# chechaohp/gan-ode

Hardware: AMD Instinct MI355X
Metric: generated videos/sec (16-frame clips) (higher is better)
Workload: dtype f32

## Files before the change

gan-ode_amd/_lib.py:

```python
from __future__ import annotations

import ctypes as C
import os

_HERE = os.path.dirname(os.path.abspath(__file__))
LIB_PATH = os.path.join(_HERE, "lib", "libgode.so")

i32, i64, f32, ptr = C.c_int32, C.c_int64, C.c_float, C.c_void_p
cint, u32, u64 = C.c_int, C.c_uint32, C.c_uint64

ACT_NONE, ACT_RELU, ACT_LRELU, ACT_TANH_OUT = 0, 1, 2, 3
ACT_TANH, ACT_SIGMOID = 4, 5
ACT_LRELU01 = 6
EPI_RAW, EPI_TANH = 0, 1
FPROP, DGRAD = 0, 1
PACK_BORDER = 0x100
OP_IGEMM, OP_WGRAD, OP_BN_FINALIZE, OP_BN_BWD, OP_ODE_FWD, OP_ODE_BWD, OP_BCE, OP_ADAM, OP_PACK = range(1, 10)
OP_ODERNN_FWD, OP_ODERNN_BWD, OP_BN_APPLY, OP_COL2IM = 10, 11, 12, 13
OP_SDE_FWD, OP_SDE_BWD = 14, 15
OP_CDE_FWD, OP_CDE_BWD = 16, 17
OP_WGAN = 18
OP_GRU_FWD, OP_GRU_BWD = 19, 20
OP_DNOISE = 21
OP_CATEG, OP_CE = 22, 23
# ... 235 lines not shown

class SnBwdOp(_Op):
    _fields_ = [("G", ptr), ("wbar", ptr), ("u", ptr), ("v", ptr), ("sigma", ptr), ("dwbar", ptr), ("work", ptr), ("h", i32),
                ("w", i32)]
    KIND, FN = OP_SN_BWD, "gode_sn_bwd"


class FcActOp(_Op):
    _fields_ = [("y", ptr), ("b", ptr), ("out", ptr), ("M", i64), ("C", i32), ("act", i32), ("key", i64), ("layer", i32),
                ("p", f32)]
    KIND, FN = OP_FC_ACT, "gode_fc_act"


class FcActBwdOp(_Op):
    _fields_ = [("g_out", ptr), ("out", ptr), ("g_y", ptr), ("db", ptr), ("work", ptr), ("M", i64), ("C", i32), ("act", i32),
                ("key", i64), ("layer", i32), ("p", f32), ("accumulate", i32), ("pad_", i32)]
    KIND, FN = OP_FC_ACT_BWD, "gode_fc_act_bwd"


class BceProbOp(_Op):
    _fields_ = [("p", ptr), ("t", ptr), ("grad", ptr), ("loss", ptr), ("n", i64), ("gscale", f32), ("accumulate", i32)]
    KIND, FN = OP_BCE_PROB, "gode_bce_prob"


class BceTOp(_Op):
    _fields_ = [("logits", ptr), ("target", ptr), ("grad", ptr), ("loss", ptr), ("n", i64), ("gscale", f32), ("accumulate", i32)]
    KIND, FN = OP_BCE_T, "gode_bce_logits_t"


class AdamNoiseTensor(C.Structure):
    _fields_ = [("p", ptr), ("g", ptr), ("m", ptr), ("v", ptr), ("n", i64), ("noise_off", i64)]


class AdamOp(_Op):
    _fields_ = [("p", ptr), ("g", ptr), ("m", ptr), ("v", ptr), ("n", i64), ("lr", f32), ("beta1", f32),
                ("beta2", f32), ("eps", f32), ("weight_decay", f32), ("gscale", f32), ("step", i32), ("pad_", i32)]
    KIND, FN = OP_ADAM, "gode_adam_l2"


class PackOp(C.Structure):
    _fields_ = [("g", ConvGeom), ("dir", i32), ("co_canon", i32), ("w", ptr), ("wpack", ptr), ("co_perm", ptr)]
    KIND = OP_PACK


_OPS = _Op.__subclasses__()
_STRUCTS = {0: ConvGeom, REC_ADAM_NOISE: AdamNoiseTensor, OP_PACK: PackOp, **{st.KIND: st for st in _OPS}}

_PROTOS = {
    "gode_igemm_stats_rows": ([ptr], cint),
    "gode_igemm_stats_rows0": ([ptr], cint),
    "gode_igemm_stats_segments": ([ptr, i32, ptr], cint),
    "gode_igemm_model_cycles": ([ptr], C.c_double),
    "gode_igemm_family": ([ptr], cint),
    "gode_igemm_work_size": ([ptr], i64),
    "gode_pack_size": ([ptr, cint], i64),
    "gode_pack_weights": ([ptr, cint, ptr, ptr, ptr, i32, ptr], cint),
    "gode_wgrad_work_size": ([ptr], i64),
    "gode_wgrad_auto_splits": ([ptr], cint),
    "gode_bn_bwd_work_size": ([i64, i32], i64),
    "gode_ode_bwd_work_size": ([i32], i64),
    "gode_odernn_bwd_work_size": ([i32], i64),
    "gode_odernn_sync_size": ([i32], i64),
    "gode_sde_bwd_work_size": ([i32], i64),
    "gode_cde_sync_size": ([i32], i64),
    "gode_cde_state_size": ([i32, i32], i64),
    "gode_cde_bwd_work_size": ([i32], i64),
    "gode_gru_bwd_work_size": ([i32], i64),
    "gode_ode_fwd_multi": ([ptr, i32, ptr], cint),
    "gode_ode_bwd_multi": ([ptr, i32, ptr], cint),
    "gode_odernn_fwd_multi": ([ptr, i32, ptr], cint),
    "gode_odernn_bwd_multi": ([ptr, i32, ptr], cint),
    "gode_gru_fwd_multi": ([ptr, i32, ptr], cint),
    "gode_gru_bwd_multi": ([ptr, i32, ptr], cint),
    "gode_chstats_rows": ([i64], cint),
    "gode_cbn_bwd_work_size": ([i32, i32, i32, i32], i64),
    "gode_gres_out_bwd_work_size": ([i32, i32, i32, i32, i32, i32], i64),
    "gode_fc_act_bwd_work_size": ([i64, i32], i64),
    "gode_dropout_mask": ([ptr, i64, u64, u32, f32, ptr], cint),
    "gode_scale": ([ptr, ptr, i64, f32, cint, ptr], cint),
    "gode_adam_multi": ([ptr, i32, i64, f32, f32, f32, f32, f32, f32, i32, ptr], cint),
    "gode_adam_multi_dev": ([ptr, i32, i64, f32, f32, f32, f32, f32, ptr, ptr], cint),
    "gode_adam_noise_multi": ([ptr, i32, i64, f32, f32, f32, f32, f32, f32, i32, u64, u32, u32, f32, ptr], cint),
    "gode_adam_noise_multi_dev": ([ptr, i32, i64, f32, f32, f32, f32, f32, ptr, u64, u32, f32, ptr], cint),
    "gode_param_noise": ([ptr, i64, u64, u32, u32, i64, f32, i32, ptr], cint),
    "gode_dnoise_normals": ([ptr, i64, u64, u32, u32, u32, i64, i32, ptr], cint),
    "gode_ode_step_chunks": ([ptr, i64], i64),
    "gode_ode_step": ([ptr, i32, i64, i32, f32, f32, f32, f32, f32, ptr, ptr], cint),
    "gode_axpy_multi": ([ptr, i32, i64, f32, ptr, ptr, f32, ptr, ptr, ptr], cint),
    "gode_run": ([ptr, ptr, i32, ptr], cint),
    "gode_version": (None, cint),
    "gode_sizeof": ([cint], cint),
}

EXPORTS = [st.FN for st in _OPS] + list(_PROTOS)

_lib = None


def lib():
    global _lib
    if _lib is not None:
        return _lib
    if not os.path.exists(LIB_PATH):
        raise RuntimeError(f"{LIB_PATH} is missing: build it with `python __graft_entry__.py` "
                           "(hipcc --offload-arch=gfx950); there is no CPU or PyTorch fallback")
    L = C.CDLL(LIB_PATH)
# ... 65 lines not shown
```

gan-ode_amd/csrc/igemm.hip:

```cpp
#include <stdlib.h>
#include "common.h"
#include "conv_geom.h"
#include "igemm_plan.h"

int gode_launch_conv_patch_fprop(const gode_igemm_op* op, const int64_t* gs, hipStream_t st);

struct IgemmArgs {
  IgemmGeom G;
  const float* src;
  const float* w;
  float* out;
  const float* scale;
  const float* shift;
  float* stats;
  int32_t gsN, gsD, gsH, gsW, gsC;
  int32_t act, epilogue;
  int32_t MB, NB, xcd_mode;
  int32_t tapskip, dmajor;
  int32_t stagger;
  int32_t ksplit, slabs_per_split;
  float* work;
  int32_t out_numel;
  int32_t stats_rows;
  uint32_t src_bytes, w_bytes;
  int32_t ntab;
  int32_t tile0[GODE_MAX_PHASES + 1];
};

__device__ __forceinline__ void igemm_block_id(const IgemmArgs& a, int& mblk, int& nblk, int& phase, int& split) {
  if (a.ntab > 0) {
    const int id = blockIdx.x;
    int p = 0;
    while (p + 1 < a.ntab && id >= a.tile0[p + 1]) ++p;
    const int t = id - a.tile0[p], NB = a.NB, mb = (a.tile0[p + 1] - a.tile0[p]) / NB;
    const int grp = t / (8 * NB), r = t - grp * 8 * NB, rest = mb - grp * 8;
    if (rest >= 8) { mblk = grp * 8 + (r & 7); nblk = r >> 3; }
    else { mblk = grp * 8 + r % rest; nblk = r / rest; }
    phase = p; split = 0;
    return;
  }
  const int MB = a.MB, NC = a.NB * a.G.nphase;
  split = blockIdx.x / (MB * NC);
  const int id = blockIdx.x - split * (MB * NC);
  int combo;
  if (a.xcd_mode == 1) {
    const int x = id & 7, j = id >> 3;
    if ((NC & 7) == 0) { combo = x + 8 * (j / MB); mblk = j % MB; }
    else { const int parts = 8 / NC; combo = x % NC; mblk = j * parts + x / NC; }
  } else if (a.xcd_mode == 2) {
    const int x = id & 7, j = id >> 3;
    combo = j % NC; mblk = (j / NC) * 8 + x;
  } else if (a.xcd_mode == 3) {
    const int x = id & 7, j = id >> 3;
    combo = j % NC; mblk = x * (MB >> 3) + j / NC;
  } else {
    mblk = id % MB; combo = id / MB;
  }
  nblk = combo % a.NB; phase = combo / a.NB;
}

template <int WM, int WN, int TM, int TN, bool VEC>
__global__ void __launch_bounds__(WM* WN * 64) igemm_kernel(const IgemmArgs a) {
  constexpr int NT = WM * WN * 64, BM = WM * TM * 32, BN = WN * TN * 32, LDK = 36;
  constexpr int RPP = NT / 8;
  constexpr int AP = BM / RPP, BP = BN / RPP;
  static_assert(BM % RPP == 0 && BN % RPP == 0, "tile/loader mismatch");
  constexpr int BUF = (BM + BN) * LDK;
  __shared__ __attribute__((aligned(16))) float smem[2 * BUF + BM * 5];
  int* rowinfo = reinterpret_cast<int*>(smem + 2 * BUF);
  int* outoff = rowinfo + BM * 4;

  const PhaseGeom& P = a.G.ph[blockIdx.z];
  const int mblk = blockIdx.x, nblk = blockIdx.y;
  if (mblk * BM >= P.M) return;
  const int tid = threadIdx.x, lane = tid & 63, wave = tid >> 6;
  const int wm = wave / WN, wn = wave % WN;
  const int Cg = a.G.Cg, Ncols = a.G.Ncols;

  for (int r = tid; r < BM; r += NT) {
    const int m = mblk * BM + r;
    int base = -1, bd = 0, bh = 0, bw = 0, oo = -1;
    if (m < P.M) {
      const int qw = m % P.Mw; int t = m / P.Mw;
      const int qh = t % P.Mh; t /= P.Mh;
      const int qd = t % P.Md; const int img = t / P.Md + P.img0;
      base = img * a.gsN;
      bd = qd * a.G.Sd + P.Od; bh = qh * a.G.Sh + P.Oh; bw = qw * a.G.Sw + P.Ow;
      oo = (((img * a.G.Xd + qd * a.G.OSd + P.Pd) * a.G.Xh + qh * a.G.OSh + P.Ph) * a.G.Xw + qw * a.G.OSw + P.Pw) *
           Ncols;
    }
    rowinfo[r * 4 + 0] = base; rowinfo[r * 4 + 1] = bd; rowinfo[r * 4 + 2] = bh; rowinfo[r * 4 + 3] = bw;
// ... 809 lines not shown
  const float neg = gode_act_neg_slope(a.act);
  const bool xf = a.scale != nullptr;
  const int64_t wave_id = (int64_t)blockIdx.x * 4 + (threadIdx.x >> 6), nwaves = (int64_t)gridDim.x * 4;
  for (int64_t m0 = wave_id * ppw; m0 < P.M; m0 += nwaves * ppw) {
    const int m = (int)m0 + sub;
    if (m >= P.M) continue;
    const uint32_t t1 = fdiv((uint32_t)m, d.dMw[0]), qw = m - t1 * P.Mw;
    const uint32_t t2 = fdiv(t1, d.dMh[0]), qh = t1 - t2 * P.Mh;
    const uint32_t img = fdiv(t2, d.dMd[0]), qd = t2 - img * P.Md;
    const int bd = (int)qd * a.G.Sd + P.Od, bh = (int)qh * a.G.Sh + P.Oh, bw = (int)qw * a.G.Sw + P.Ow;
    f32x4 acc = {0.f, 0.f, 0.f, 0.f};
    int k = 0;
    for (int jd = 0; jd < P.Td; ++jd)
      for (int jh = 0; jh < P.Th; ++jh)
        for (int jw = 0; jw < P.Tw; ++jw) {
          const int id = bd + a.G.J * jd, ih = bh + a.G.J * jh, iw = bw + a.G.J * jw;
          const bool ok = (unsigned)id < (unsigned)a.G.Gd && (unsigned)ih < (unsigned)a.G.Gh && (unsigned)iw < (unsigned)a.G.Gw;
          const int off = (int)img * a.gsN + id * a.gsD + ih * a.gsH + iw * a.gsW;
          for (int c = 0; c < Cg; ++c, ++k) {
            float v = 0.f;
            if (ok) {
              v = a.src[off + c * a.gsC];
              if (xf) v = v * a.scale[c] + a.shift[c];
              v = fmaxf(v, v * neg);
            }
            const f32x4 w = *reinterpret_cast<const f32x4*>(wl + k * Ncols + c4);
            acc[0] += v * w[0]; acc[1] += v * w[1]; acc[2] += v * w[2]; acc[3] += v * w[3];
          }
        }
    const int oo = ((((int)img * a.G.Xd + (int)qd * a.G.OSd + P.Pd) * a.G.Xh + (int)qh * a.G.OSh + P.Ph) * a.G.Xw +
                    (int)qw * a.G.OSw + P.Pw) * Ncols;
    if (a.epilogue == GODE_EPI_TANH) { acc[0] = tanhf(acc[0]); acc[1] = tanhf(acc[1]); acc[2] = tanhf(acc[2]); acc[3] = tanhf(acc[3]); }
    *reinterpret_cast<f32x4*>(a.out + oo + c4) = acc;
  }
}

extern "C" int gode_igemm_stats_rows0(const gode_igemm_op* op) {
  IgemmPlan P;
  const int rc = igemm_make_plan(op, &P);
  return rc ? rc : P.rows0;
}

extern "C" double gode_igemm_model_cycles(const gode_igemm_op* op) {
  IgemmPlan P;
  return igemm_make_plan(op, &P) ? -1.0 : P.cycles;
}

extern "C" int gode_igemm_family(const gode_igemm_op* op) {
  IgemmPlan P;
  const int rc = igemm_make_plan(op, &P);
  return rc ? rc : P.family;
}

extern "C" int gode_igemm_stats_segments(const gode_igemm_op* op, int32_t split_images, int32_t* seg) {
  if (!op || !seg || op->groups == 2 || op->border || split_images <= 0 || split_images >= op->g.N) return GODE_E_ARG;
  IgemmPlan P;
  const int rc = igemm_make_plan(op, &P);
  if (rc) return rc;
  if (P.ksplit > 1) {
    const int64_t per_img = (int64_t)P.G.Xd * P.G.Xh * P.G.Xw;
    const int64_t b = (int64_t)split_images * per_img;
    if (b % SPLITK_ROWS != 0) return GODE_E_SHAPE;
    seg[0] = 0; seg[1] = (int32_t)(b / SPLITK_ROWS); seg[2] = P.stats_rows;
    return 1;
  }
  const int bm = tile_bm(P.tile);
  for (int i = 0; i < P.G.nphase; ++i) {
    const PhaseGeom& Ph = P.G.ph[i];
    const int64_t per_img = (int64_t)Ph.Md * Ph.Mh * Ph.Mw;
    const int64_t b = (int64_t)split_images * per_img;
    if (Ph.M != (int64_t)op->g.N * per_img) return GODE_E_SHAPE;
    if (b % bm != 0) return GODE_E_SHAPE;
    seg[3 * i] = Ph.row0; seg[3 * i + 1] = Ph.row0 + (int32_t)(b / bm); seg[3 * i + 2] = Ph.row0 + gode_ceil_div(Ph.M, bm);
  }
  return P.G.nphase;
}

extern "C" int gode_igemm_stats_rows(const gode_igemm_op* op) {
  IgemmPlan P;
  const int rc = igemm_make_plan(op, &P);
  return rc ? rc : P.stats_rows;
}

extern "C" int64_t gode_igemm_work_size(const gode_igemm_op* op) {
  IgemmPlan P;
  const int rc = igemm_make_plan(op, &P);
  if (rc) return rc;
  return P.ksplit > 1 ? (int64_t)P.ksplit * P.positions * P.G.Ncols : 0;
}

template <int TILE>
static int launch(IgemmArgs& A, const IgemmPlan& P, bool vec, hipStream_t st) {
  constexpr IgemmTile T = IGEMM_TILES[TILE];
  constexpr int WM = T.WM, WN = T.WN, TM = T.TM, TN = T.TN;
  dim3 grid(P.max_mblk, gode_ceil_div(A.G.Ncols, T.bn), A.G.nphase), block(WM * WN * 64);
  const bool fast = vec && P.fast;
  if (P.ksplit > 1 && (!fast || A.work == nullptr)) return GODE_E_ARG;
  if (fast) {
    static const char* senv = getenv("GODE_IGEMM_STAGGER");
    A.stagger = senv ? atoi(senv) : 0;
#ifndef GODE_ABLATION_BUILD
    if (A.stagger < 0) A.stagger = 0;
#endif
    const dim3 g1(P.ntab > 0 ? P.tile0[P.ntab] : P.MB * P.NB * A.G.nphase * P.ksplit);
    const bool has_xf = A.scale != nullptr || A.act != GODE_ACT_NONE;
    const bool glds = !has_xf && A.src_bytes != 0 && A.w_bytes != 0;
// ... 8 lines not shown
                           dim3(256), 0, st, A.work, A.out, A.stats, P.positions, A.G.Ncols, P.ksplit, A.epilogue);
      else
        hipLaunchKernelGGL(igemm_splitk_reduce_kernel, dim3(gode_ceil_div(P.positions, SPLITK_ROWS)), dim3(256), 0, st, A.work, A.out,
                           A.stats, P.positions, A.G.Ncols, P.ksplit, A.epilogue);
    }
  }
  else if (vec) hipLaunchKernelGGL((igemm_kernel<WM, WN, TM, TN, true>), grid, block, 0, st, A);
  else hipLaunchKernelGGL((igemm_kernel<WM, WN, TM, TN, false>), grid, block, 0, st, A);
  GODE_LAUNCH_CHECK();
  return 0;
}

static PwArgs pw_args(const IgemmArgs& A, int lanes_per_position) {
  PwArgs D; D.a = A; D.lpp = lanes_per_position;
  for (int i = 0; i < A.G.nphase; ++i) {
    D.dMw[i] = make_fastdiv((uint32_t)A.G.ph[i].Mw); D.dMh[i] = make_fastdiv((uint32_t)A.G.ph[i].Mh);
    D.dMd[i] = make_fastdiv((uint32_t)A.G.ph[i].Md);
  }
  return D;
}

extern "C" int gode_igemm(const gode_igemm_op* op, void* stream) {
  if (!op || !op->src || !op->wpack || !op->out) return GODE_E_ARG;
  IgemmPlan P;
  int rc = igemm_make_plan(op, &P);
  if (rc) return rc;
  if (P.max_mblk == 0) return 0;
  const IgemmGeom& G = P.G;
  int64_t gs[5];
  if (gode_strides_are_channels_last(op->gs)) {
    gs[4] = 1; gs[3] = G.Cg; gs[2] = (int64_t)G.Gw * gs[3]; gs[1] = (int64_t)G.Gh * gs[2]; gs[0] = (int64_t)G.Gd * gs[1];
  } else {
    for (int i = 0; i < 5; ++i) gs[i] = op->gs[i];
  }
  int64_t span = 1 + (int64_t)(op->g.N - 1) * gs[0] + (int64_t)(G.Gd - 1) * gs[1] + (int64_t)(G.Gh - 1) * gs[2] +
                 (int64_t)(G.Gw - 1) * gs[3] + (int64_t)(G.Cg - 1) * gs[4];
  int64_t outn = (int64_t)op->g.N * G.Xd * G.Xh * G.Xw * G.Ncols;
  for (int i = 0; i < 5; ++i) if (gs[i] < 0) return GODE_E_ARG;
  if (span >= (1ll << 31) || outn >= (1ll << 31)) return GODE_E_SHAPE;
  if (((uintptr_t)op->wpack % 16) != 0 || (op->scale == nullptr) != (op->shift == nullptr)) return GODE_E_ARG;
  hipStream_t st = (hipStream_t)stream;
  if (P.family == IGEMM_PATCH_FPROP) {
    const int pr = gode_launch_conv_patch_fprop(op, gs, st);
    if (pr != 0) return pr < 0 ? pr : 0;
  }
  IgemmArgs A;
  A.G = G;
  A.src = op->src; A.w = op->wpack; A.out = op->out; A.scale = op->scale; A.shift = op->shift; A.stats = op->stats;
  A.gsN = (int)gs[0]; A.gsD = (int)gs[1]; A.gsH = (int)gs[2]; A.gsW = (int)gs[3]; A.gsC = (int)gs[4];
  A.act = op->act; A.epilogue = op->epilogue;
  A.stagger = 0;
  A.tapskip = P.tapskip; A.dmajor = P.dmajor; A.stats_rows = P.stats_rows;
  A.ksplit = P.ksplit; A.slabs_per_split = P.slabs_per_split;
  A.MB = P.MB; A.NB = P.NB; A.xcd_mode = P.xcd_mode; A.ntab = P.ntab;
  for (int i = 0; i <= GODE_MAX_PHASES; ++i) A.tile0[i] = P.tile0[i];
  A.src_bytes = span * 4 < (1ll << 31) ? (uint32_t)(span * 4) : 0u;
  A.w_bytes = gode_pack_floats(G) * 4 < (1ll << 31) ? (uint32_t)(gode_pack_floats(G) * 4) : 0u;
  A.work = op->work; A.out_numel = (int32_t)outn;
  const bool vec = P.vec && ((uintptr_t)op->src % 16) == 0 &&
                   (op->scale == nullptr || ((uintptr_t)op->scale % 16 == 0 && (uintptr_t)op->shift % 16 == 0));
  int maxM = 0, minK = 1 << 30;
  for (int i = 0; i < G.nphase; ++i) {
    if (G.ph[i].M > maxM) maxM = G.ph[i].M;
    if (G.ph[i].K < minK) minK = G.ph[i].K;
  }
  if (P.family == IGEMM_POINTWISE && vec) {
    const int lpp = G.Cg / 4;
    const bool one_tap = G.nphase == 1 && G.ph[0].K == G.Cg;
    const PwArgs D = pw_args(A, lpp);
    int64_t blocks = ((int64_t)maxM + (64 / lpp) * 4 * 8 - 1) / ((64 / lpp) * 4 * 8);
    if (blocks > (one_tap ? 4096 : 2048)) blocks = one_tap ? 4096 : 2048;
    if (one_tap && G.Ncols == 1 && lpp <= 16) {
      const int64_t its = ((int64_t)maxM + (64 / lpp) * PW1_U - 1) / ((64 / lpp) * PW1_U), per_wave = (its + 8191) / 8192;
      const dim3 g1((unsigned)((its + 4 * per_wave - 1) / (4 * per_wave)));
      if (lpp == 16) hipLaunchKernelGGL(conv_pointwise1_kernel<16>, g1, dim3(256), 0, st, D);
      else if (lpp == 8) hipLaunchKernelGGL(conv_pointwise1_kernel<8>, g1, dim3(256), 0, st, D);
      else hipLaunchKernelGGL(conv_pointwise1_kernel<4>, g1, dim3(256), 0, st, D);
    }
    else if (one_tap) hipLaunchKernelGGL(conv_pointwise_kernel<true>, dim3((int)blocks, 1), dim3(256), 0, st, D);
    else hipLaunchKernelGGL(conv_pointwise_kernel<false>, dim3((int)blocks, G.nphase), dim3(256), 0, st, D);
  } else if (P.family == IGEMM_SMALLK && ((uintptr_t)op->out % 16) == 0) {
    const int nl = G.Ncols / 4;
    const PwArgs D = pw_args(A, nl);
    int64_t blocks = ((int64_t)maxM + (64 / nl) * 4 * 4 - 1) / ((64 / nl) * 4 * 4);
    if (blocks > 4096) blocks = 4096;
    hipLaunchKernelGGL(conv_smallk_kernel, dim3((int)blocks), dim3(256), 0, st, D);
  } else if (P.family == IGEMM_DOT && vec) {
    DotArgs D; D.a = A; D.dCg = make_fastdiv((uint32_t)G.Cg);
    D.per_block = (maxM <= 256 && minK >= 4096) ? 1 : 4;
    hipLaunchKernelGGL(conv_dot_kernel, dim3(D.per_block == 1 ? maxM : gode_ceil_div(maxM, 4), G.nphase), dim3(256), 0, st, D);
  } else {
    static int (*const launchers[IGEMM_TILE_IDS])(IgemmArgs&, const IgemmPlan&, bool, hipStream_t) = {
        nullptr, launch<TILE_128x128>, launch<TILE_128x64>, launch<TILE_128x32>, launch<TILE_64x64>, nullptr, launch<TILE_256x128>};
    return launchers[P.tile](A, P, vec, st);
  }
  GODE_LAUNCH_CHECK();
  return 0;
}

struct PackArgs {
  IgemmGeom G;
  gode_conv_geom g;
  int dir;
  const float* w;
  float* wp;
  const int32_t* co_perm;
};
// ... 213 lines not shown
```

gan-ode_amd/csrc/igemm_plan.h:

```cpp
#pragma once
#include <stdio.h>
#include <stdlib.h>
#include "conv_geom.h"

#define IGEMM_MAX_LIVE_TAPS 64
#define SPLITK_ROWS 16
#define PW_MAXW 4096

enum { TILE_128x128 = 1, TILE_128x64 = 2, TILE_128x32 = 3, TILE_64x64 = 4, TILE_256x128 = 6, IGEMM_TILE_IDS = 7 };
struct IgemmTile { int bm, bn, WM, WN, TM, TN; double cps; int resident; double eff2; };
constexpr IgemmTile igemm_tile(int WM, int WN, int TM, int TN, double cps, int resident, double eff2) {
  return IgemmTile{WM * TM * 32, WN * TN * 32, WM, WN, TM, TN, cps, resident, eff2};
}
static constexpr IgemmTile IGEMM_TILES[IGEMM_TILE_IDS] = {
    igemm_tile(0, 0, 0, 0, 0.0, 0, 0.0),
    igemm_tile(2, 2, 2, 2, 4096.0, 2, 0.76),
    igemm_tile(2, 2, 2, 1, 2048.0, 3, 0.76),
    igemm_tile(4, 1, 1, 1, 1024.0, 4, 0.62),
    igemm_tile(2, 2, 1, 1, 1024.0, 4, 0.70),
    igemm_tile(0, 0, 0, 0, 0.0, 0, 0.0),
    igemm_tile(4, 2, 2, 2, 8192.0, 1, 0.785)};

static bool tile_exists(int tile) { return tile > 0 && tile < IGEMM_TILE_IDS && IGEMM_TILES[tile].bm != 0; }
static int tile_bm(int tile) { return IGEMM_TILES[tile].bm; }
// ... 98 lines not shown
      if (cyc < best * 0.97) { best = cyc; best_tile = t; best_k = k; }
    }
  }
  *cycles_out = best;
  if (live_taps) {
    const int64_t t128 = count_tiles(G, TILE_128x128), t64 = count_tiles(G, TILE_64x64);
    if (t128 < 256 && G.Ncols >= 64 && min_slabs == max_slabs) {
      int k = (int)((1152 + t64 / 2) / t64);
      if (k < 1) k = 1;
      while (k > 1 && (min_slabs / k < 8 || out_bytes * k > 192e6)) --k;
      best_tile = TILE_64x64; best_k = k;
    }
  }
  *tile_out = best_tile;
  *sp_out = split_k(op, G, max_slabs, best_k);
}

static bool border_table(const gode_igemm_op* op, const IgemmGeom& G, IgemmGeom* B) {
  if (!op->border || op->dir != GODE_DGRAD || op->groups == 2 || G.fullk || igemm_wants_tapskip(op, G)) return false;
  return gode_build_igemm_geom_border(op->g, op->dir, B) == 0 && B->border != 0;
}

#define BORDER_LOSS 1.06
static void choose_border(const IgemmGeom& B, int* tile_out, double* cycles_out) {
  static const int tiles[2] = {TILE_128x64, TILE_64x64};
  double best = 1e300; int best_tile = TILE_128x64;
  for (int ti = 0; ti < 2; ++ti) {
    const int t = tiles[ti], bm = tile_bm(t), bn = tile_bn(t);
    if (bn >= 2 * B.Ncols && bn > 32) continue;
    const double cps = IGEMM_TILES[t].cps, eff = IGEMM_TILES[t].eff2;
    const int resident = IGEMM_TILES[t].resident;
    if (3 * count_tiles(B, t) < 4 * 256 * (int64_t)resident) continue;
    double work = 0;
    for (int i = 0; i < B.nphase; ++i)
      work += (double)gode_ceil_div(B.ph[i].M, bm) * gode_ceil_div(B.Ncols, bn) * (4000.0 + (B.ph[i].K >> 5) * cps / eff);
    const double cyc = BORDER_LOSS * work / 256.0;
    if (cyc < best) { best = cyc; best_tile = t; }
  }
  *tile_out = best_tile; *cycles_out = best;
}

enum { IGEMM_GEMM = 0, IGEMM_PATCH_FPROP = 1, IGEMM_POINTWISE = 2, IGEMM_SMALLK = 3, IGEMM_DOT = 4 };

struct IgemmPlan {
  IgemmGeom G;
  int32_t family;
  int32_t tile;
  int32_t vec, fast;
  int32_t ksplit, slabs_per_split, positions;
  int32_t max_mblk, stats_rows, rows0;
  int32_t tapskip, dmajor;
  int32_t xcd_mode, MB, NB;
  int32_t ntab, tile0[GODE_MAX_PHASES + 1];
  double cycles;
};

static int thin_family(const gode_igemm_op* op, const IgemmGeom& G, bool vec) {
  if (op->tile != 0 || op->stats != nullptr || op->groups == 2) return IGEMM_GEMM;
  if (op->dir == GODE_FPROP && !op->scale && !op->shift && op->act == GODE_ACT_NONE && op->epilogue == GODE_EPI_RAW && op->g.Ci <= 4 &&
      op->g.Co >= 32 && G.ph[0].K >= 8)
    return IGEMM_PATCH_FPROP;
  int maxM = 0, minK = 1 << 30, maxK = 0; bool kp_ok = true;
  for (int i = 0; i < G.nphase; ++i) {
    if (G.ph[i].M > maxM) maxM = G.ph[i].M;
    if (G.ph[i].K < minK) minK = G.ph[i].K;
    if (G.ph[i].Kp > maxK) maxK = G.ph[i].Kp;
    kp_ok = kp_ok && G.ph[i].Kp == G.ph[i].K;
  }
  const int lpp = G.Cg / 4, nl = G.Ncols / 4;
  const bool one_tap = G.nphase == 1 && G.ph[0].K == G.Cg;
  if (vec && kp_ok && G.Ncols <= 4 && G.Ncols * maxK <= PW_MAXW && maxM >= (one_tap ? 4096 : 65536) &&
      (lpp == 4 || lpp == 8 || lpp == 16 || lpp == 32 || lpp == 64))
    return IGEMM_POINTWISE;
  if (G.nphase == 1 && G.ph[0].K <= 4 && G.Ncols % 4 == 0 && G.Ncols <= 128 && maxM >= 2048 && (nl == 4 || nl == 8 || nl == 16 || nl == 32))
    return IGEMM_SMALLK;
  if (vec && kp_ok && G.Ncols <= 4 && maxM <= 16384 && minK >= 512) return IGEMM_DOT;
  return IGEMM_GEMM;
}

static void plan_grid_order(const gode_igemm_op* op, IgemmPlan* P) {
  const IgemmGeom& G = P->G;
  P->MB = 0; P->NB = 0; P->xcd_mode = 0; P->ntab = 0;
  for (int i = 0; i <= GODE_MAX_PHASES; ++i) P->tile0[i] = 0;
  if (!P->fast) return;
  const int MB = P->max_mblk, NB = gode_ceil_div(G.Ncols, tile_bn(P->tile)), NC = NB * G.nphase;
  P->MB = MB; P->NB = NB;
  static const char* xenv = getenv("GODE_IGEMM_XCD");
  const int force = xenv ? atoi(xenv) : -1;
  const int64_t wbytes = gode_pack_floats(G) * 4;
  const bool ok1 = (NC % 8 == 0) || (NC < 8 && 8 % NC == 0 && MB % (8 / NC) == 0);
  const bool ok2 = MB % 8 == 0;
  const int64_t in_bytes = (int64_t)op->g.N * G.Gd * G.Gh * G.Gw * G.Cg * 4;
  int mode = ok2 ? (wbytes * 8 < 3 * in_bytes ? 3 : 0) : 0;
  if (P->dmajor > 0) mode = ok2 ? 2 : (ok1 ? 1 : 0);
  if (force == 0) mode = 0;
  if (force == 1 && ok1) mode = 1;
  if (force == 2 && ok2) mode = 2;
  if (force == 3 && ok2) mode = 3;
  P->xcd_mode = mode;
  if (G.border) {
    P->ntab = G.nphase;
    for (int i = 0; i < G.nphase; ++i) P->tile0[i + 1] = P->tile0[i] + gode_ceil_div(G.ph[i].M, tile_bm(P->tile)) * NB;
    for (int i = G.nphase + 1; i <= GODE_MAX_PHASES; ++i) P->tile0[i] = P->tile0[G.nphase];
  }
}

static int igemm_make_plan(const gode_igemm_op* op, IgemmPlan* P) {
  if (!op || (op->tile != 0 && !tile_exists(op->tile))) return GODE_E_ARG;
  IgemmGeom& G = P->G;
  int rc = gode_build_igemm_geom(op->g, op->dir, &G);
  if (rc) return rc;
  P->tapskip = igemm_wants_tapskip(op, G);
  P->dmajor = P->tapskip ? op->g.N : 0;
  IgemmGeom B;
  const bool can_border = border_table(op, G, &B);
  const bool grouped = op->groups == 2;
  if (grouped) {
    if (op->dir != GODE_FPROP || op->g.N % 2 != 0 || G.nphase != 1) return GODE_E_ARG;
    G.ph[1] = G.ph[0];
    G.ph[0].M /= 2; G.ph[1].M = G.ph[0].M; G.ph[1].img0 = op->g.N / 2;
    G.nphase = 2;
  } else if (op->groups != 0 && op->groups != 1) return GODE_E_ARG;
  P->vec = strides_allow_vec(op, G);
  int tile; SplitPlan sp; double cyc = -1.0;
  bool take_border = false;
  if (op->tile == 0 && fast_geometry(G) && G.Ncols > 4 && P->vec) {
    choose_fast(op, G, &tile, &sp, &cyc);
    if (can_border && fast_geometry(B) && sp.ksplit == 1) {
      int tb; double cb;
      choose_border(B, &tb, &cb);
      if (cb < 0.97 * cyc) { take_border = true; tile = tb; cyc = cb; }
    }
    static const bool sweeping = getenv("GODE_IGEMM_SWEEP") != nullptr;
    const char* fenv = sweeping ? getenv("GODE_IGEMM_FORCE") : nullptr;
    int fk = 0, min_slabs, max_slabs;
    if (fenv && sscanf(fenv, "%d,%d", &tile, &fk) == 2) {
      if (!tile_exists(tile)) return GODE_E_ARG;
      slab_range(G, &min_slabs, &max_slabs);
      sp = split_k(op, G, max_slabs, fk);
      take_border = can_border && fk <= 1;
    }
  } else {
    tile = pick_tile(G, op->tile);
    sp = plan_split(op, G, tile);
    if (can_border && sp.ksplit == 1 && op->tile != 0) {
      const int tb = pick_tile(B, op->tile);
      const SplitPlan sb = plan_split(op, B, tb);
      if (sb.ksplit == 1) { take_border = true; tile = tb; sp = sb; }
    }
  }
  if (take_border) G = B;
  if (grouped && sp.ksplit > 1 && (sp.positions / 2) % SPLITK_ROWS != 0) {
    sp.ksplit = 1; sp.slabs_per_split = 0;
  }
  const int bm = tile_bm(tile);
  int r0 = 0, mx = 0;
  for (int i = 0; i < G.nphase; ++i) {
    G.ph[i].row0 = r0;
    const int mb = gode_ceil_div(G.ph[i].M, bm);
    r0 += mb;
    if (mb > mx) mx = mb;
  }
  P->tile = tile; P->ksplit = sp.ksplit; P->slabs_per_split = sp.slabs_per_split; P->positions = sp.positions;
  P->max_mblk = mx;
  P->stats_rows = sp.ksplit > 1 ? gode_ceil_div(sp.positions, SPLITK_ROWS) : r0;
  P->rows0 = !grouped ? P->stats_rows : (sp.ksplit > 1 ? P->stats_rows / 2 : G.ph[1].row0);
  P->cycles = grouped ? -1.0 : cyc;
  P->fast = P->vec && fast_geometry(G);
  P->family = thin_family(op, G, P->vec);
  plan_grid_order(op, P);
  return 0;
}
```

gan-ode_amd/engine.py:

```python
from __future__ import annotations

import ctypes as C
import os
from dataclasses import dataclass
from typing import List, Optional, Sequence

import numpy as np
import torch

from . import _lib as L


def make_geom(N, Ci, Co, xi, yo, k, s, p) -> L.ConvGeom:
    return L.ConvGeom(N, Ci, Co, xi[0], xi[1], xi[2], yo[0], yo[1], yo[2], k[0], k[1], k[2], s[0], s[1], s[2],
                      p[0], p[1], p[2])


def conv_out(i, k, s, p):
    return (i + 2 * p - k) // s + 1


def dptr(t: Optional[torch.Tensor]):
    return None if t is None else t.data_ptr()


def stream_ptr():
    return torch.cuda.current_stream().cuda_stream


@dataclass
class LayerSpec:
    geom: L.ConvGeom
    fwd_dir: int
    act: int
    has_bn: bool
    epilogue: int = L.EPI_RAW
    co_perm: Optional[torch.Tensor] = None
    noise: bool = False

    def out_dims(self):
        g = self.geom
        if self.fwd_dir == L.FPROP:
            return (g.N, g.Do, g.Ho, g.Wo, g.Co)
        return (g.N, g.Di, g.Hi, g.Wi, g.Ci)

    def in_dims(self):
        g = self.geom
        if self.fwd_dir == L.FPROP:
            return (g.N, g.Di, g.Hi, g.Wi, g.Ci)
        return (g.N, g.Do, g.Ho, g.Wo, g.Co)


@dataclass
class LayerParams:
    weight: torch.Tensor
    gamma: Optional[torch.Tensor] = None
    beta: Optional[torch.Tensor] = None
    running_mean: Optional[torch.Tensor] = None
    running_var: Optional[torch.Tensor] = None
    num_batches_tracked: Optional[torch.Tensor] = None


def _contig_strides(dims):
    n, d, h, w, c = dims
    return (d * h * w * c, h * w * c, w * c, c, 1)


class ConvStack:

    def __init__(self, specs: Sequence[LayerSpec], params: Sequence[LayerParams], device, owns_input: bool,
                 momentum=0.1, eps=1e-5, pack_cache: Optional[dict] = None, groups: int = 1, split_images: int = 0,
                 split_order: int = 0, two_lane_backward: bool = False):
        self.specs, self.params, self.device = list(specs), list(params), device
        self.groups = groups
        self.two_lane = bool(two_lane_backward)
        self._lane_stream = None
        self.split, self.split_order = int(split_images), int(split_order)
        if self.split and (groups != 1 or not owns_input or not (0 < self.split < specs[0].geom.N)):
            raise ValueError("split ConvStack: plan-owned input, one launch group, 0 < split_images < N")
        self._G2 = groups == 2 or self.split > 0
        self._last_parts = False
        if groups not in (1, 2) or (groups == 2 and (owns_input or specs[0].fwd_dir != L.FPROP or specs[0].has_bn
                                                     or specs[0].geom.N % 2)):
            raise ValueError("grouped ConvStack: two groups, Conv stack, caller-owned input, no BatchNorm on layer 0")
        self.nl = len(specs)
        self.noisy = any(s.noise for s in specs)
        if self.noisy and (owns_input or self.split):
            raise ValueError("instance noise: caller-owned input, no split stack")
        self.momentum, self.eps = momentum, eps
        self.busy = False
        self.generation = 0
        self._fwd_training = True
        self.pack_cache = pack_cache if pack_cache is not None else {}
        lib = L.lib()
        f32 = dict(dtype=torch.float32, device=device)
        self.x_in = torch.zeros(specs[0].in_dims(), **f32) if owns_input else None
        self.x0n = torch.empty(specs[0].in_dims(), **f32) if specs[0].noise else None
        self.y = [torch.empty(s.out_dims(), **f32) for s in specs[:-1]]
        self.a = [torch.empty(s.out_dims(), **f32) if self._materialize(l) else None for l, s in enumerate(specs[:-1])]
        self.out_dims = specs[-1].out_dims()
        self.wpack_f, self.wpack_b = [], [None] * self.nl
        self.stats, self.stat_rows = [], []
        self.mean, self.invstd, self.scale, self.shift = [], [], [], []
        self._two_f, self._two_b, self._rows_ab = {}, {}, {}
        self._border = self._border_layers() if os.environ.get("GODE_BORDER_SPLIT", "1") != "0" else {}
        for l, s in enumerate(specs):
            bord = l in self._border
            n = lib.gode_pack_size(C.byref(s.geom), s.fwd_dir | (L.PACK_BORDER if bord else 0))
            if n <= 0:
                raise RuntimeError(f"bad geometry for pack ({n})")
            self.wpack_f.append(self._shared_pack(l, "border" if bord else s.fwd_dir, n))
            C_out = s.out_dims()[4]
            two = self._two_f[l] = bool(self.split) and 0 < l < self.nl - 1 and self._two_launches(s.geom, s.fwd_dir)
            if s.has_bn:
                probe = L.IgemmOp(g=s.geom, dir=s.fwd_dir, tile=0, groups=groups, border=1 if bord else 0)
                if two:
                    ra, rb = (lib.gode_igemm_stats_rows(C.byref(L.IgemmOp(g=self._part_geom(s.geom, n), dir=s.fwd_dir, tile=0)))
                              for n in (self.split, s.geom.N - self.split))
                    rows = ra + rb if ra > 0 and rb > 0 else -1
                    self._rows_ab[l] = (ra, rb)
                else:
                    rows = lib.gode_igemm_stats_rows(C.byref(probe))
                if rows <= 0:
                    raise RuntimeError(f"layer {l}: no partial-statistics layout for this geometry ({rows})")
                ncols = self._ncols(s)
                self.stat_rows.append(rows)
                self.stats.append(torch.empty(rows * 2 * ncols, **f32))
                ng = 2 if self._G2 else 1
                self.mean.append(torch.empty(ng * C_out, **f32)); self.invstd.append(torch.empty(ng * C_out, **f32))
                self.scale.append(torch.empty(ng * C_out, **f32)); self.shift.append(torch.empty(ng * C_out, **f32))
                if self.split and not two:
                    seg = (C.c_int32 * 24)()
                    nseg = lib.gode_igemm_stats_segments(C.byref(probe), self.split, seg)
                    if nseg <= 0:
                        raise ValueError(f"layer {l}: the statistics rows do not split at image {self.split} ({nseg})")
                    self.__dict__.setdefault("_segs", {})[l] = (nseg, list(seg))
            else:
                self.stat_rows.append(0); self.stats.append(None)
                self.mean.append(None); self.invstd.append(None); self.scale.append(None); self.shift.append(None)
        self._ig_work = None
        self._fwd = {}
        self._bwd = {}
        self.g = None
        self._param_ptrs = None

    def _shared_pack(self, l, direction, n):
        key = ("buf", l, direction)
        buf = self.pack_cache.get(key)
        if buf is None or buf.numel() != n or buf.device != torch.device(self.device):
            buf = self.pack_cache[key] = torch.empty(n, dtype=torch.float32, device=self.device)
            self.pack_cache.pop(("ver", l, direction), None)
        return buf

    def _attach_work(self, igemm_ops):
        lib = L.lib()
        need = max([lib.gode_igemm_work_size(C.byref(op)) for op in igemm_ops] + [0])
        if need > 0:
            if self._ig_work is None or self._ig_work.numel() < need:
                self._ig_work = torch.empty(need, dtype=torch.float32, device=self.device)
                for prog_ops in getattr(self, "_all_igemm", []):
                    for op in prog_ops:
                        op.work = self._ig_work.data_ptr()
            for op in igemm_ops:
                op.work = self._ig_work.data_ptr()
        self.__dict__.setdefault("_all_igemm", []).append(list(igemm_ops))

    def _run_stale_packs(self, packs, st):
        stale = []
# ... 175 lines not shown
                wp = self._shared_pack(l, "head_gemm", n)
                packs.append((l, "head_gemm", L.PackOp(g=hg, dir=L.DGRAD, co_canon=0, w=dptr(p.weight), wpack=dptr(wp),
                                                       co_perm=dptr(s.co_perm))))
                g = s.geom
                if getattr(self, "_head_cols", None) is None:
                    self._head_cols = torch.empty(hg.N * g.kh * g.kw * g.Ci, dtype=torch.float32, device=self.device)
                if self._last_parts:
                    pix, Cs = g.Ho * g.Wo, sc.numel() // 2
                    for n, img0, k in ((self.split, 0, 0), (g.N - self.split, self.split, 1)):
                        pg = self._part_geom(hg, n * pix)
                        ops.append(L.IgemmOp(g=pg, dir=L.DGRAD, act=act, epilogue=L.EPI_RAW, tile=0,
                                             src=src.data_ptr() + 4 * img0 * pix * g.Co, wpack=dptr(wp),
                                             out=self._head_cols.data_ptr() + 4 * img0 * pix * g.kh * g.kw * g.Ci,
                                             scale=sc.data_ptr() + 4 * Cs * k, shift=sh.data_ptr() + 4 * Cs * k))
                else:
                    ops.append(L.IgemmOp(g=hg, dir=L.DGRAD, act=act, epilogue=L.EPI_RAW, tile=0, src=dptr(src), wpack=dptr(wp),
                                         out=dptr(self._head_cols), scale=dptr(sc), shift=dptr(sh)))
                c2i = L.Col2imOp(cols=dptr(self._head_cols), out=None, N=g.N, Hi=g.Ho, Wi=g.Wo, Ho=g.Hi, Wo=g.Wi, C=g.Ci,
                                 kh=g.kh, kw=g.kw, sh=g.sh, sw=g.sw, ph=g.ph, pw=g.pw, epilogue=s.epilogue)
                ops.append(c2i)
                patch["last"] = c2i
                if l == 0:
                    raise RuntimeError("a one-layer stack cannot use the GEMM + col2im head")
                continue
            want_stats = s.has_bn and training
            if self._last_parts and l == self.nl - 1:
                per_in, per_out, Cs = int(np.prod(s.in_dims()[1:])), int(np.prod(s.out_dims()[1:])), sc.numel() // 2
                pair = []
                for n, img0, k in ((self.split, 0, 0), (s.geom.N - self.split, self.split, 1)):
                    pair.append(L.IgemmOp(g=self._part_geom(s.geom, n), dir=s.fwd_dir, act=act, epilogue=s.epilogue, tile=0,
                                          src=src.data_ptr() + 4 * img0 * per_in, wpack=dptr(self.wpack_f[l]), out=None,
                                          scale=sc.data_ptr() + 4 * Cs * k, shift=sh.data_ptr() + 4 * Cs * k))
                ops += pair
                patch["last"], patch["last2"] = pair[0], (pair[1], 4 * self.split * per_out)
                continue
            if self._two_f.get(l):
                ra = self._rows_ab[l][0] if s.has_bn else 0
                per_in, per_out = int(np.prod(s.in_dims()[1:])), int(np.prod(s.out_dims()[1:]))
                for n, img0, st_off in ((self.split, 0, 0), (s.geom.N - self.split, self.split, ra * 2 * self._ncols(s))):
                    ops.append(L.IgemmOp(g=self._part_geom(s.geom, n), dir=s.fwd_dir, act=act, epilogue=s.epilogue, tile=0,
                                         src=src.data_ptr() + 4 * img0 * per_in, wpack=dptr(self.wpack_f[l]),
                                         out=self.y[l].data_ptr() + 4 * img0 * per_out, scale=dptr(sc), shift=dptr(sh),
                                         stats=self.stats[l].data_ptr() + 4 * st_off if want_stats else None, groups=0))
                op = None
            else:
                op = L.IgemmOp(g=s.geom, dir=s.fwd_dir, act=act, epilogue=s.epilogue, tile=0, src=dptr(src),
                               wpack=dptr(self.wpack_f[l]), out=dptr(self.y[l]) if l < self.nl - 1 else None,
                               scale=dptr(sc), shift=dptr(sh),
                               stats=dptr(self.stats[l]) if want_stats else None,
                               groups=2 if (G2 and s.has_bn) else 0)
                if l in self._border:
                    packs[-1] = (l, "border", L.PackOp(g=s.geom, dir=L.DGRAD | L.PACK_BORDER, co_canon=0, w=dptr(p.weight),
                                                       wpack=dptr(self.wpack_f[l]), co_perm=dptr(s.co_perm)))
                    op.border = 1
                ops.append(op)
            if l == 0:
                patch["first"] = op
            if l == self.nl - 1:
                patch["last"] = op
            if s.has_bn:
                rows0 = lib.gode_igemm_stats_rows0(C.byref(op)) if G2 else 0
                fin = L.BnFinalizeOp(stats=dptr(self.stats[l]), rows=self.stat_rows[l], ncols=self._ncols(s),
                                     C=s.out_dims()[4], count=self._count(l) // self.groups, gamma=dptr(p.gamma),
                                     beta=dptr(p.beta), running_mean=dptr(p.running_mean),
                                     running_var=dptr(p.running_var),
                                     num_batches_tracked=dptr(p.num_batches_tracked), mean=dptr(self.mean[l]),
                                     invstd=dptr(self.invstd[l]), scale=dptr(self.scale[l]),
                                     shift=dptr(self.shift[l]), momentum=self.momentum, eps=self.eps,
                                     training=1 if training else 0, groups=self.groups if G2 else 0, rows0=rows0)
                if self.split:
                    per_img = self._count(l) // s.geom.N
                    fin.groups, fin.order = 2, self.split_order
                    fin.count, fin.count1 = per_img * self.split, per_img * (s.geom.N - self.split)
                    if self._two_f.get(l):
                        ra, rb = self._rows_ab[l]
                        fin.rows, fin.rows1 = ra, rb
                        fin.stats1 = self.stats[l].data_ptr() + 4 * ra * 2 * self._ncols(s)
                    else:
                        nseg, seg = self._segs[l]
                        fin.nseg = nseg
                        for k in range(3 * nseg):
                            fin.seg[k] = seg[k]
                ops.append(fin)
            if l < self.nl - 1 and self.a[l] is not None:
                d = s.out_dims()
                M = d[0] * d[1] * d[2] * d[3]
                M0 = M // 2 if (G2 and s.has_bn) else ((M // d[0]) * self.split if (self.split and s.has_bn) else 0)
                if self.specs[l + 1].noise:
                    ops.append(self._noise_op(noise, l, dptr(self.scale[l]), dptr(self.shift[l]), M // 2 if G2 else 0))
                    continue
                ops.append(L.BnApplyOp(y=dptr(self.y[l]), out=dptr(self.a[l]), scale=dptr(self.scale[l]),
                                       shift=dptr(self.shift[l]), M=M, C=d[4], act=s.act, M0=M0))
        patch["packs"] = packs
        self._attach_work([op for op in ops if isinstance(op, L.IgemmOp)])
        return L.Program(ops), patch

    def _noise_op(self, noise, l, scale, shift, M0):
        d = self.specs[l].out_dims()
        op = L.DnoiseOp(x=dptr(self.y[l]), out=dptr(self.a[l]), scale=scale, shift=shift, M=d[0] * d[1] * d[2] * d[3],
                        C=d[4], act=self.specs[l].act, M0=M0, layer=l + 1)
        noise.append((op, d[1] * d[2] * d[3] * d[4], 0, None))
        return op

    @staticmethod
    def _patch_noise(patch, noise, inputs):
        seed = int(noise["seed"]) & 0xFFFFFFFFFFFFFFFF
        seed = seed - (1 << 64) if seed >= 1 << 63 else seed
# ... 308 lines not shown
```

include/gode.h:

```cpp
#ifndef GODE_H
#define GODE_H
#include <stdint.h>
#ifdef __cplusplus
extern "C" {
#endif

#define GODE_VERSION 105

enum { GODE_OK = 0, GODE_E_ARG = -1, GODE_E_SHAPE = -2, GODE_E_KIND = -3 };
enum { GODE_ACT_NONE = 0, GODE_ACT_RELU = 1, GODE_ACT_LRELU = 2,
       GODE_ACT_TANH_OUT = 3 ,
       GODE_ACT_TANH = 4, GODE_ACT_SIGMOID = 5 ,
       GODE_ACT_LRELU01 = 6  };
enum { GODE_EPI_RAW = 0, GODE_EPI_TANH = 1 };
enum { GODE_FPROP = 0, GODE_DGRAD = 1 };
enum { GODE_PACK_BORDER = 0x100 };

typedef struct gode_conv_geom {
  int32_t N, Ci, Co;
  int32_t Di, Hi, Wi;
  int32_t Do, Ho, Wo;
  int32_t kd, kh, kw;
  int32_t sd, sh, sw;
  int32_t pd, ph, pw;
} gode_conv_geom;

typedef struct gode_igemm_op {
  gode_conv_geom g;
  int32_t dir, act, epilogue, tile;
  const float* src;
  const float* wpack;
  float* out;
  const float* scale;
  const float* shift;
  float* stats;
  int64_t gs[5];
  float* work;
  int32_t groups;
  int32_t border;
} gode_igemm_op;
int gode_igemm(const gode_igemm_op* op, void* stream);
int64_t gode_igemm_work_size(const gode_igemm_op* op);
int gode_igemm_stats_rows(const gode_igemm_op* op);
int gode_igemm_stats_rows0(const gode_igemm_op* op);
int gode_igemm_stats_segments(const gode_igemm_op* op, int32_t split_images, int32_t* seg);
double gode_igemm_model_cycles(const gode_igemm_op* op);
int gode_igemm_family(const gode_igemm_op* op);
int64_t gode_pack_size(const gode_conv_geom* g, int dir);
int gode_pack_weights(const gode_conv_geom* g, int dir, const float* w, float* wpack, const int32_t* co_perm,
                      int32_t co_canon, void* stream);

typedef struct gode_wgrad_op {
  gode_conv_geom g;
  int32_t act, xform_on_y, splits, accumulate;
  const float* x;
  const float* y;
  const float* scale;
  const float* shift;
  float* work;
  float* dw;
  const int32_t* co_perm; int64_t co_canon;
  int64_t xs[5];
} gode_wgrad_op;
int gode_wgrad(const gode_wgrad_op* op, void* stream);
int64_t gode_wgrad_work_size(const gode_wgrad_op* op);
int gode_wgrad_auto_splits(const gode_conv_geom* g);

typedef struct gode_bn_finalize_op {
  const float* stats; int32_t rows, ncols, C; int64_t count;
  const float* gamma; const float* beta;
  float* running_mean; float* running_var; int64_t* num_batches_tracked;
  float* mean; float* invstd; float* scale; float* shift;
  float momentum, eps; int32_t training, pad_;
  int32_t groups, rows0;
  int32_t nseg, order; int64_t count1; int32_t seg[24];
  const float* stats1; int32_t rows1, pad3_;
} gode_bn_finalize_op;
int gode_bn_finalize(const gode_bn_finalize_op* op, void* stream);

typedef struct gode_bn_apply_op {
  const float* y; float* out; const float* scale; const float* shift; int64_t M; int32_t C, act;
  int64_t M0;
} gode_bn_apply_op;
int gode_bn_apply(const gode_bn_apply_op* op, void* stream);

typedef struct gode_col2im_op {
  const float* cols; float* out;
  int32_t N, Hi, Wi, Ho, Wo, C, kh, kw, sh, sw, ph, pw;
  int32_t epilogue, pad_;
  int32_t Di, Do, kd, sd, pd, pad2_;
} gode_col2im_op;
int gode_col2im(const gode_col2im_op* op, void* stream);

typedef struct gode_bn_bwd_op {
  float* g; const float* y; int64_t M; int32_t C, act;
  const float* gamma; const float* mean; const float* invstd; const float* scale; const float* shift;
  float* dgamma; float* dbeta; float* work; int32_t accumulate, eval_mode;
  const float* gin;
  int32_t groups, pad2_;
  int64_t M0;
// ... 328 lines not shown
```

Baseline: 37580.

## Force border-split igemm when dead taps are significant and interleave phase classes

Adds a border=2 mode that is chosen per layer from the fraction of dead taps and the tile count relative to resident slots. In that mode the planner takes the border (tap-skipping) decomposition unconditionally instead of only when the cycle model predicts a gain. It also reorders the phases into classes with matching shapes and interleaves the spatial residues inside each grid segment. The intent is to skip the zero-tap work in transposed convolutions and keep the grid balanced. The risk is overriding the cost model where the border split is slower, and it adds more indexing arithmetic to the block-id mapping.

```diff
diff --git a/gan-ode_amd/_lib.py b/gan-ode_amd/_lib.py
--- a/gan-ode_amd/_lib.py
+++ b/gan-ode_amd/_lib.py
@@ -311,6 +311,8 @@
     "gode_igemm_stats_segments": ([ptr, i32, ptr], cint),
     "gode_igemm_model_cycles": ([ptr], C.c_double),
     "gode_igemm_family": ([ptr], cint),
+    "gode_igemm_dead_taps": ([ptr], C.c_double),
+    "gode_igemm_launch_info": ([ptr, ptr], cint),
     "gode_igemm_work_size": ([ptr], i64),
     "gode_pack_size": ([ptr, cint], i64),
     "gode_pack_weights": ([ptr, cint, ptr, ptr, ptr, i32, ptr], cint),
diff --git a/gan-ode_amd/csrc/igemm.hip b/gan-ode_amd/csrc/igemm.hip
--- a/gan-ode_amd/csrc/igemm.hip
+++ b/gan-ode_amd/csrc/igemm.hip
@@ -23,20 +23,14 @@
   int32_t out_numel;
   int32_t stats_rows;
   uint32_t src_bytes, w_bytes;
-  int32_t ntab;
+  int32_t ntab, interleave;
   int32_t tile0[GODE_MAX_PHASES + 1];
 };
 
 __device__ __forceinline__ void igemm_block_id(const IgemmArgs& a, int& mblk, int& nblk, int& phase, int& split) {
   if (a.ntab > 0) {
-    const int id = blockIdx.x;
-    int p = 0;
-    while (p + 1 < a.ntab && id >= a.tile0[p + 1]) ++p;
-    const int t = id - a.tile0[p], NB = a.NB, mb = (a.tile0[p + 1] - a.tile0[p]) / NB;
-    const int grp = t / (8 * NB), r = t - grp * 8 * NB, rest = mb - grp * 8;
-    if (rest >= 8) { mblk = grp * 8 + (r & 7); nblk = r >> 3; }
-    else { mblk = grp * 8 + r % rest; nblk = r / rest; }
-    phase = p; split = 0;
+    igemm_border_block(blockIdx.x, a.ntab, a.tile0, a.NB, a.interleave, mblk, nblk, phase);
+    split = 0;
     return;
   }
   const int MB = a.MB, NC = a.NB * a.G.nphase;
@@ -952,6 +946,29 @@
   return rc ? rc : P.family;
 }
 
+extern "C" double gode_igemm_dead_taps(const gode_igemm_op* op) {
+  if (!op) return 0.0;
+  gode_igemm_op flagged = *op;
+  flagged.border = 1;
+  IgemmGeom G, B;
+  if (gode_build_igemm_geom(op->g, op->dir, &G) || !border_table(&flagged, G, &B)) return 0.0;
+  double plain = 0, live = 0;
+  for (int i = 0; i < G.nphase; ++i) plain += (double)G.ph[i].M * G.ph[i].K;
+  for (int i = 0; i < B.nphase; ++i) live += (double)B.ph[i].M * B.ph[i].K;
+  return plain > 0 ? 1.0 - live / plain : 0.0;
+}
+
+extern "C" int gode_igemm_launch_info(const gode_igemm_op* op, int32_t* info) {
+  if (!info) return GODE_E_ARG;
+  IgemmPlan P;
+  const int rc = igemm_make_plan(op, &P);
+  if (rc) return rc;
+  info[0] = P.G.border != 0; info[1] = P.tile;
+  info[2] = P.ntab > 0 ? P.tile0[P.ntab] : (int32_t)count_tiles(P.G, P.tile) * P.ksplit;
+  info[3] = 256 * IGEMM_TILES[P.tile].resident;
+  return 0;
+}
+
 extern "C" int gode_igemm_stats_segments(const gode_igemm_op* op, int32_t split_images, int32_t* seg) {
   if (!op || !seg || op->groups == 2 || op->border || split_images <= 0 || split_images >= op->g.N) return GODE_E_ARG;
   IgemmPlan P;
@@ -1066,7 +1083,7 @@
   A.stagger = 0;
   A.tapskip = P.tapskip; A.dmajor = P.dmajor; A.stats_rows = P.stats_rows;
   A.ksplit = P.ksplit; A.slabs_per_split = P.slabs_per_split;
-  A.MB = P.MB; A.NB = P.NB; A.xcd_mode = P.xcd_mode; A.ntab = P.ntab;
+  A.MB = P.MB; A.NB = P.NB; A.xcd_mode = P.xcd_mode; A.ntab = P.ntab; A.interleave = P.interleave;
   for (int i = 0; i <= GODE_MAX_PHASES; ++i) A.tile0[i] = P.tile0[i];
   A.src_bytes = span * 4 < (1ll << 31) ? (uint32_t)(span * 4) : 0u;
   A.w_bytes = gode_pack_floats(G) * 4 < (1ll << 31) ? (uint32_t)(gode_pack_floats(G) * 4) : 0u;
diff --git a/gan-ode_amd/csrc/igemm_plan.h b/gan-ode_amd/csrc/igemm_plan.h
--- a/gan-ode_amd/csrc/igemm_plan.h
+++ b/gan-ode_amd/csrc/igemm_plan.h
@@ -174,6 +174,7 @@
   int32_t tapskip, dmajor;
   int32_t xcd_mode, MB, NB;
   int32_t ntab, tile0[GODE_MAX_PHASES + 1];
+  int32_t interleave;
   double cycles;
 };
 
@@ -200,9 +201,42 @@
   return IGEMM_GEMM;
 }
 
+GODE_HD void igemm_border_block(int id, int ntab, const int32_t* tile0, int NB, int np, int& mblk, int& nblk, int& phase) {
+  int e = 0;
+  while (e + 1 < ntab && id >= tile0[e + 1]) ++e;
+  const int NC = NB * np, t = id - tile0[e], mb = (tile0[e + 1] - tile0[e]) / NC;
+  const int grp = t / (8 * NC), r = t - grp * 8 * NC, rest = mb - grp * 8;
+  int combo;
+  if (rest >= 8) { mblk = grp * 8 + (r & 7); combo = r >> 3; }
+  else { mblk = grp * 8 + r % rest; combo = r / rest; }
+  nblk = combo % NB; phase = e * np + combo / NB;
+}
+
+static int border_classes(const IgemmGeom& B, int order[GODE_MAX_PHASES]) {
+  const int nsp = B.OSd * B.OSh * B.OSw;
+  if (!B.border || nsp < 2 || B.nphase % nsp != 0) return 0;
+  const int ncls = B.nphase / nsp;
+  int rep[GODE_MAX_PHASES], count[GODE_MAX_PHASES], seen[GODE_MAX_PHASES], nc = 0;
+  for (int i = 0; i < B.nphase; ++i) {
+    const PhaseGeom& s = B.ph[i];
+    int c = 0;
+    for (; c < nc; ++c) {
+      const PhaseGeom& r = B.ph[rep[c]];
+      if (r.Md == s.Md && r.Mh == s.Mh && r.Mw == s.Mw && r.Td == s.Td && r.Th == s.Th && r.Tw == s.Tw) break;
+    }
+    if (c == nc) { if (nc == ncls) return 0; rep[nc] = i; count[nc] = 0; seen[nc] = 0; ++nc; }
+    const int residue = ((s.Pd % B.OSd) * B.OSh + s.Ph % B.OSh) * B.OSw + s.Pw % B.OSw;
+    if (count[c] == nsp || (seen[c] >> residue & 1)) return 0;
+    seen[c] |= 1 << residue;
+    order[c * nsp + count[c]++] = i;
+  }
+  for (int c = 0; c < nc; ++c) if (count[c] != nsp) return 0;
+  return nc == ncls ? nsp : 0;
+}
+
 static void plan_grid_order(const gode_igemm_op* op, IgemmPlan* P) {
-  const IgemmGeom& G = P->G;
-  P->MB = 0; P->NB = 0; P->xcd_mode = 0; P->ntab = 0;
+  IgemmGeom& G = P->G;
+  P->MB = 0; P->NB = 0; P->xcd_mode = 0; P->ntab = 0; P->interleave = 0;
   for (int i = 0; i <= GODE_MAX_PHASES; ++i) P->tile0[i] = 0;
   if (!P->fast) return;
   const int MB = P->max_mblk, NB = gode_ceil_div(G.Ncols, tile_bn(P->tile)), NC = NB * G.nphase;
@@ -221,9 +255,18 @@
   if (force == 3 && ok2) mode = 3;
   P->xcd_mode = mode;
   if (G.border) {
-    P->ntab = G.nphase;
-    for (int i = 0; i < G.nphase; ++i) P->tile0[i + 1] = P->tile0[i] + gode_ceil_div(G.ph[i].M, tile_bm(P->tile)) * NB;
-    for (int i = G.nphase + 1; i <= GODE_MAX_PHASES; ++i) P->tile0[i] = P->tile0[G.nphase];
+    int order[GODE_MAX_PHASES];
+    static const char* oenv = getenv("GODE_IGEMM_BORDER_ORDER");
+    const int np = op->border == 2 && !(oenv && atoi(oenv) == 0) ? border_classes(G, order) : 0;
+    if (np > 0) {
+      const IgemmGeom T = G;
+      for (int i = 0; i < G.nphase; ++i) G.ph[i] = T.ph[order[i]];
+    }
+    P->interleave = np > 0 ? np : 1;
+    P->ntab = G.nphase / P->interleave;
+    for (int e = 0; e < P->ntab; ++e)
+      P->tile0[e + 1] = P->tile0[e] + gode_ceil_div(G.ph[e * P->interleave].M, tile_bm(P->tile)) * NB * P->interleave;
+    for (int i = P->ntab + 1; i <= GODE_MAX_PHASES; ++i) P->tile0[i] = P->tile0[P->ntab];
   }
 }
 
@@ -251,7 +294,7 @@
     if (can_border && fast_geometry(B) && sp.ksplit == 1) {
       int tb; double cb;
       choose_border(B, &tb, &cb);
-      if (cb < 0.97 * cyc) { take_border = true; tile = tb; cyc = cb; }
+      if (op->border == 2 ? cb < 1e300 : cb < 0.97 * cyc) { take_border = true; tile = tb; cyc = cb; }
     }
     static const bool sweeping = getenv("GODE_IGEMM_SWEEP") != nullptr;
     const char* fenv = sweeping ? getenv("GODE_IGEMM_FORCE") : nullptr;
@@ -265,7 +308,7 @@
   } else {
     tile = pick_tile(G, op->tile);
     sp = plan_split(op, G, tile);
-    if (can_border && sp.ksplit == 1 && op->tile != 0) {
+    if (can_border && sp.ksplit == 1 && op->tile != 0 && (op->border != 2 || (P->vec && fast_geometry(G) && fast_geometry(B)))) {
       const int tb = pick_tile(B, op->tile);
       const SplitPlan sb = plan_split(op, B, tb);
       if (sb.ksplit == 1) { take_border = true; tile = tb; sp = sb; }
diff --git a/gan-ode_amd/engine.py b/gan-ode_amd/engine.py
--- a/gan-ode_amd/engine.py
+++ b/gan-ode_amd/engine.py
@@ -9,6 +9,18 @@
 import torch
 
 from . import _lib as L
+
+BORDER_TAKE_DEAD_TAPS = 0.06
+BORDER_TAKE_TILES_PER_SLOT = 2.0
+
+
+def border_value(g) -> int:
+    lib = L.lib()
+    if lib.gode_igemm_dead_taps(C.byref(L.IgemmOp(g=g, dir=L.DGRAD, tile=0))) < BORDER_TAKE_DEAD_TAPS:
+        return 1
+    info = (C.c_int32 * 4)()
+    L.check(lib.gode_igemm_launch_info(C.byref(L.IgemmOp(g=g, dir=L.DGRAD, tile=0, border=2)), info))
+    return 2 if info[0] and info[2] >= BORDER_TAKE_TILES_PER_SLOT * info[3] else 1
 
 
 def make_geom(N, Ci, Co, xi, yo, k, s, p) -> L.ConvGeom:
@@ -104,8 +116,9 @@
         self.mean, self.invstd, self.scale, self.shift = [], [], [], []
         self._two_f, self._two_b, self._rows_ab = {}, {}, {}
         self._border = self._border_layers() if os.environ.get("GODE_BORDER_SPLIT", "1") != "0" else {}
+        self._border_flag = {l: border_value(specs[l].geom) for l in self._border}
         for l, s in enumerate(specs):
-            bord = l in self._border
+            bord = self._border_flag.get(l, 0)
             n = lib.gode_pack_size(C.byref(s.geom), s.fwd_dir | (L.PACK_BORDER if bord else 0))
             if n <= 0:
                 raise RuntimeError(f"bad geometry for pack ({n})")
@@ -113,7 +126,7 @@
             C_out = s.out_dims()[4]
             two = self._two_f[l] = bool(self.split) and 0 < l < self.nl - 1 and self._two_launches(s.geom, s.fwd_dir)
             if s.has_bn:
-                probe = L.IgemmOp(g=s.geom, dir=s.fwd_dir, tile=0, groups=groups, border=1 if bord else 0)
+                probe = L.IgemmOp(g=s.geom, dir=s.fwd_dir, tile=0, groups=groups, border=bord)
                 if two:
                     ra, rb = (lib.gode_igemm_stats_rows(C.byref(L.IgemmOp(g=self._part_geom(s.geom, n), dir=s.fwd_dir, tile=0)))
                               for n in (self.split, s.geom.N - self.split))
@@ -395,7 +408,7 @@
                 if l in self._border:
                     packs[-1] = (l, "border", L.PackOp(g=s.geom, dir=L.DGRAD | L.PACK_BORDER, co_canon=0, w=dptr(p.weight),
                                                        wpack=dptr(self.wpack_f[l]), co_perm=dptr(s.co_perm)))
-                    op.border = 1
+                    op.border = self._border_flag[l]
                 ops.append(op)
             if l == 0:
                 patch["first"] = op
diff --git a/include/gode.h b/include/gode.h
--- a/include/gode.h
+++ b/include/gode.h
@@ -46,6 +46,8 @@
 int gode_igemm_stats_segments(const gode_igemm_op* op, int32_t split_images, int32_t* seg);
 double gode_igemm_model_cycles(const gode_igemm_op* op);
 int gode_igemm_family(const gode_igemm_op* op);
+double gode_igemm_dead_taps(const gode_igemm_op* op);
+int gode_igemm_launch_info(const gode_igemm_op* op, int32_t* info);
 int64_t gode_pack_size(const gode_conv_geom* g, int dir);
 int gode_pack_weights(const gode_conv_geom* g, int dir, const float* w, float* wpack, const int32_t* co_perm,
                       int32_t co_canon, void* stream);
```

New measurement: 38670 (median of 6 runs). 2.9% higher.
